# ShenhanQian/GaussianAvatars

Hardware: NVIDIA H100
Metric: rasterizer fwd+bwd frames/sec @100k splats 1080p (higher is better)
Workload: dtype f32

## Files before the change

gaussianavatars_b200/csrc/blend.cu:

```cuda
#include <type_traits>

#include "common.cuh"
#include "kernels.cuh"

namespace gab {

#define LOG2E 1.4426950408889634f
#define ALPHA_MIN (1.0f / 255.0f)
#define FULLMASK 0xffffffffu
#define CONIC_UNSCALE_AC (-2.0f / LOG2E)
#define CONIC_UNSCALE_B (-1.0f / LOG2E)

__device__ __forceinline__ float ex2_approx(float x) {
  float y;
  asm("ex2.approx.ftz.f32 %0, %1;" : "=f"(y) : "f"(x));
  return y;
}
__device__ __forceinline__ float rcp_approx(float x) {
  float y;
  asm("rcp.approx.ftz.f32 %0, %1;" : "=f"(y) : "f"(x));
  return y;
}
__device__ __forceinline__ void cp_async16(void* smem_dst, const void* gmem_src) {
  const unsigned s = (unsigned)__cvta_generic_to_shared(smem_dst);
  asm volatile("cp.async.cg.shared.global [%0], [%1], 16;" ::"r"(s), "l"(gmem_src) : "memory");
}
__device__ __forceinline__ void cp_async_commit() { asm volatile("cp.async.commit_group;" ::: "memory"); }
template <int N>
__device__ __forceinline__ void cp_async_wait() {
  asm volatile("cp.async.wait_group %0;" ::"n"(N) : "memory");
}
__device__ __forceinline__ void gather_rec(SplatRec* dst, const SplatRec* src) {
  cp_async16(&dst->q0, &src->q0);
  cp_async16(&dst->q1, &src->q1);
  cp_async16(&dst->q2, &src->q2);
}

__device__ __forceinline__ uint32_t smem_u32(const void* p) { return (uint32_t)__cvta_generic_to_shared(p); }
__device__ __forceinline__ void mbar_init(uint64_t* bar, uint32_t count) {
  asm volatile("mbarrier.init.shared::cta.b64 [%0], %1;" ::"r"(smem_u32(bar)), "r"(count) : "memory");
}
__device__ __forceinline__ void mbar_fence_init() { asm volatile("fence.mbarrier_init.release.cluster;" ::: "memory"); }
__device__ __forceinline__ void mbar_arrive_expect_tx(uint64_t* bar, uint32_t bytes) {
  asm volatile("mbarrier.arrive.expect_tx.shared::cta.b64 _, [%0], %1;" ::"r"(smem_u32(bar)), "r"(bytes) : "memory");
}
__device__ __forceinline__ void bulk_copy_g2s(void* smem_dst, const void* gmem_src, uint32_t bytes, uint64_t* bar) {
  asm volatile("cp.async.bulk.shared::cluster.global.mbarrier::complete_tx::bytes [%0], [%1], %2, [%3];" ::"r"(
                   smem_u32(smem_dst)),
               "l"(gmem_src), "r"(bytes), "r"(smem_u32(bar))
               : "memory");
}
__device__ __forceinline__ void mbar_wait(uint64_t* bar, uint32_t parity) {
  asm volatile(
      "{\n\t.reg .pred p;\n\tMBAR_WAIT:\n\tmbarrier.try_wait.parity.shared::cta.b64 p, [%0], %1;\n\t@p bra MBAR_DONE;\n\t"
      "bra MBAR_WAIT;\n\tMBAR_DONE:\n\t}" ::"r"(smem_u32(bar)),
      "r"(parity)
      : "memory");
}
#define GAB_FWD_DEPTH_CTAS 2
#define GAB_BWD_DEPTH_CTAS 5
#define ID_RING 3

template <int NT>
struct GroupBarrier {
  int id;
  __device__ __forceinline__ void sync() const { asm volatile("bar.sync %0, %1;" ::"r"(id), "n"(NT) : "memory"); }
  __device__ __forceinline__ bool sync_and(bool pred) const {
    unsigned r;
    asm volatile(
        "{\n\t.reg .pred p, q;\n\tsetp.ne.u32 q, %1, 0;\n\tbar.red.and.pred p, %2, %3, q;\n\tselp.u32 %0, 1, 0, p;\n\t}"
        : "=r"(r)
        : "r"((unsigned)pred), "r"(id), "n"(NT)
        : "memory");
    return r != 0;
  }
};

template <int K>
struct BandGeom {
  int col, row0, half, band0;
  __device__ __forceinline__ explicit BandGeom(int tl) {
    const int w = tl >> 5, lane = tl & 31;
    half = w & 1;
    band0 = (w >> 1) * K;
    col = half * 8 + (lane & 7);
    row0 = band0 * 4 + (lane >> 3);
  }
  __device__ __forceinline__ int bit(int i) const { return 2 * (band0 + i) + half; }
};

#define BLEND_OUT_FLOAT 1
#define BLEND_OUT_U8 2
__device__ __forceinline__ uint32_t quantize_u8(float c) {
  return __float2uint_rz(fminf(fmaxf(__fadd_rn(__fmul_rn(c, 255.f), 0.5f), 0.f), 255.f));
}
__device__ __forceinline__ void store_display(uint8_t* __restrict__ out, int W, int H, int pixx, int y, int lane,
                                              float r, float g, float b) {
  const uint32_t px = quantize_u8(r) | (quantize_u8(g) << 8) | (quantize_u8(b) << 16);
  const int j = lane & 7, x0 = pixx - j;
  const int p0 = min((4 * j) / 3, 6);
  const uint32_t lo = __shfl_sync(FULLMASK, px, (lane & ~7) | p0);
  const uint32_t hi = __shfl_sync(FULLMASK, px, (lane & ~7) | (p0 + 1));
  const uint32_t word = (uint32_t)((((uint64_t)hi << 24) | lo) >> (8 * (4 * j - 3 * p0)));
  if (y >= H) return;
  const size_t row = (size_t)y * W;
  if ((W & 3) == 0 && x0 + 8 <= W && ((uintptr_t)out & 3u) == 0) {
    if (j < 6) reinterpret_cast<uint32_t*>(out)[(row + x0) / 4 * 3 + j] = word;
  } else if (pixx < W) {
    uint8_t* o = out + (row + pixx) * 3;
    o[0] = (uint8_t)px;
    o[1] = (uint8_t)(px >> 8);
    o[2] = (uint8_t)(px >> 16);
  }
}

template <int K, int OUT, bool DA = false>
__device__ __forceinline__ void forward_tile(int tile, int tl, GroupBarrier<256 / K> bar, SplatRec* buf0,
                                             SplatRec* buf1, uint32_t* smask, uint32_t* ids_ring, uint64_t* mbar,
                                             int W, int H, int gx,
                                             const uint2* __restrict__ ranges, const uint32_t* __restrict__ point_list,
                                             const SplatRec* __restrict__ rec, const float* __restrict__ bg,
                                             float* __restrict__ out_color, float* __restrict__ final_T,
                                             uint32_t* __restrict__ n_contrib, uint8_t* __restrict__ strip_mask,
                                             uint8_t* __restrict__ out_rgb8, float* __restrict__ out_alpha = nullptr,
                                             float* __restrict__ out_depth = nullptr) {
  constexpr int NT = 256 / K;
  const int tx = tile % gx, ty = tile / gx;
  const int lane = tl & 31;
  const BandGeom<K> geo(tl);
  const int pixx = tx * GAB_TILE + geo.col;
  const int pixy0 = ty * GAB_TILE + geo.row0;
  const float fx = (float)pixx;
  float fy[K];
#pragma unroll
  for (int i = 0; i < K; i++) fy[i] = (float)(pixy0 + 4 * i);
  const uint2 range = ranges[tile];
  const int n = (int)(range.y - range.x);
  const uint32_t* ids = point_list + range.x;
  const bool want_mask = strip_mask != nullptr;
  smask[tl] = 0;

  float T[K], Cr[K], Cg[K], Cb[K];
  float D[DA ? K : 1];
  uint32_t last[K];
  uint32_t done = 0;
  constexpr uint32_t ALL = (1u << K) - 1u;
#pragma unroll
  for (int i = 0; i < K; i++) {
    T[i] = 1.f; Cr[i] = Cg[i] = Cb[i] = 0.f; last[i] = 0;
    if (DA) D[i] = 0.f;
    if (pixx >= W || pixy0 + 4 * i >= H) done |= 1u << i;
  }

  const int nchunks = (n + NT - 1) / NT;
  constexpr int RING_STRIDE = NT + 4;
  constexpr uint32_t CHUNK_BYTES = RING_STRIDE * 4;
  const int mis = (int)(range.x & 3u);
  const uint32_t* ids_al = ids - mis;
  if (tl == 0) {
#pragma unroll
    for (int k = 0; k < ID_RING; k++) mbar_init(&mbar[k], 1);
    mbar_fence_init();
  }
  bar.sync();
  auto issue_ids = [&](int k) {
    uint64_t* b = &mbar[k % ID_RING];
    mbar_arrive_expect_tx(b, CHUNK_BYTES);
    bulk_copy_g2s(ids_ring + (k % ID_RING) * RING_STRIDE, ids_al + (size_t)k * NT, CHUNK_BYTES, b);
  };
  auto wait_ids = [&](int k) { mbar_wait(&mbar[k % ID_RING], (uint32_t)((k / ID_RING) & 1)); };
  if (tl == 0) {
    if (nchunks > 0) issue_ids(0);
    if (nchunks > 1) issue_ids(1);
  }
  if (nchunks > 0) {
    wait_ids(0);
    if (tl < n) gather_rec(&buf0[tl], rec + ids_ring[mis + tl]);
  }
  cp_async_commit();

  for (int c = 0; c < nchunks; c++) {
    SplatRec* nxt = ((c + 1) & 1) ? buf1 : buf0;
    if (c + 1 < nchunks) {
      wait_ids(c + 1);
      const int p = (c + 1) * NT + tl;
      if (p < n) gather_rec(&nxt[tl], rec + ids_ring[((c + 1) % ID_RING) * RING_STRIDE + mis + tl]);
    }
    cp_async_commit();
    if (tl == 0 && c + 2 < nchunks) issue_ids(c + 2);
    cp_async_wait<1>();
    if (bar.sync_and(done == ALL)) {
      if (c + 2 < nchunks) wait_ids(c + 2);
      break;
    }
    const SplatRec* cur = (c & 1) ? buf1 : buf0;
    const int cnt = min(NT, n - c * NT);
    const uint32_t pos0 = (uint32_t)(c * NT);
    uint32_t lb[K];
#pragma unroll
    for (int i = 0; i < K; i++) lb[i] = 0;
    for (int gbase = 0; gbase < cnt; gbase += 32) {
      const int gend = min(32, cnt - gbase);
#pragma unroll 4
      for (int jj = 0; jj < gend; jj++) {
        const SplatRec* r = cur + gbase + jj;
        const float4 q0 = r->q0;
        const float4 q1 = r->q1;
        const float dx = q0.x - fx;
        const float tA = q0.z * dx;
#pragma unroll
        for (int i = 0; i < K; i++) {
          const float dy = q0.y - fy[i];
          const float pw = fmaf(q1.x * dy, dy, fmaf(q0.w, dy, tA) * dx);
          const float alpha = fminf(0.99f, q1.y * ex2_approx(pw));
          if (pw <= 0.f && alpha >= ALPHA_MIN && !((done >> i) & 1u)) {
            const float test_T = T[i] * (1.f - alpha);
            if (test_T < 0.0001f) {
              done |= 1u << i;
            } else {
              const float w = alpha * T[i];
              Cr[i] = fmaf(q1.z, w, Cr[i]);
              Cg[i] = fmaf(q1.w, w, Cg[i]);
              Cb[i] = fmaf(r->q2.x, w, Cb[i]);
              if (DA) D[i] = fmaf(r->q2.w, w, D[i]);
              T[i] = test_T;
              last[i] = pos0 + (uint32_t)(gbase + jj) + 1u;
              lb[i] |= 1u << jj;
            }
          }
        }
      }
      if (want_mask) {
        uint32_t wh = 0;
#pragma unroll
        for (int i = 0; i < K; i++) {
          const uint32_t rr = __reduce_or_sync(FULLMASK, lb[i]);
          wh |= ((rr >> lane) & 1u) << geo.bit(i);
          lb[i] = 0;
        }
        if (wh) atomicOr(&smask[gbase + lane], wh);
      }
      if (__all_sync(FULLMASK, done == ALL)) break;
    }
    bar.sync();
    if (want_mask && tl < cnt) {
      strip_mask[range.x + (uint32_t)(c * NT + tl)] = (uint8_t)smask[tl];
      smask[tl] = 0;
    }
  }
  cp_async_wait<0>();

  const float bg0 = bg[0], bg1 = bg[1], bg2 = bg[2];
  const size_t HW = (size_t)H * W;
#pragma unroll
  for (int i = 0; i < K; i++) {
    const int y = pixy0 + 4 * i;
    if (pixx < W && y < H) {
      const size_t pix = (size_t)y * W + pixx;
      if (OUT & BLEND_OUT_FLOAT) {
        out_color[pix] = fmaf(T[i], bg0, Cr[i]);
        out_color[HW + pix] = fmaf(T[i], bg1, Cg[i]);
        out_color[2 * HW + pix] = fmaf(T[i], bg2, Cb[i]);
      }
      if (final_T != nullptr) {
        final_T[pix] = T[i];
        n_contrib[pix] = last[i];
      }
      if (DA) {
        if (out_alpha != nullptr) out_alpha[pix] = 1.0f - T[i];
        if (out_depth != nullptr) out_depth[pix] = D[i];
      }
    }
  }
  if (OUT & BLEND_OUT_U8) {
#pragma unroll
    for (int i = 0; i < K; i++)
      store_display(out_rgb8, W, H, pixx, pixy0 + 4 * i, lane, fmaf(T[i], bg0, Cr[i]), fmaf(T[i], bg1, Cg[i]),
                    fmaf(T[i], bg2, Cb[i]));
  }
}

template <int KH, int OUT>
__global__ void __launch_bounds__(256) blend_forward_kernel(int W, int H, int gx, int tiles,
                                                            const uint2* __restrict__ ranges,
                                                            const uint32_t* __restrict__ order,
                                                            const uint32_t* __restrict__ order_info,
                                                            const uint32_t* __restrict__ point_list,
                                                            const SplatRec* __restrict__ rec,
                                                            const float* __restrict__ bg, float* __restrict__ out_color,
                                                            float* __restrict__ final_T,
                                                            uint32_t* __restrict__ n_contrib,
                                                            uint8_t* __restrict__ strip_mask,
                                                            uint8_t* __restrict__ out_rgb8) {
  __shared__ SplatRec buf[2][256];
  __shared__ uint32_t smask[256];
  __shared__ __align__(16) uint32_t ids_ring[4][ID_RING * (64 + 4)];
  __shared__ __align__(8) uint64_t mbar[4][ID_RING];
  constexpr int GH = KH;
  constexpr int NTH = 256 / KH;
  const int nh = (int)order_info[0];
  const int heavy_ctas = (nh + GH - 1) / GH;
  const int b = blockIdx.x, t = threadIdx.x;
  if (b < heavy_ctas) {
    const int g = t / NTH, slot = b * GH + g;
    if (slot >= nh) return;
    forward_tile<KH, OUT>((int)order[slot], t - g * NTH, GroupBarrier<NTH>{GH == 1 ? 0 : 1 + g}, buf[0] + g * NTH,
                          buf[1] + g * NTH, smask + g * NTH, &ids_ring[0][0] + g * (ID_RING * (NTH + 4)), mbar[g], W,
                          H, gx, ranges, point_list, rec, bg, out_color, final_T, n_contrib, strip_mask, out_rgb8);
  } else {
    const int g = t >> 6, slot = nh + 4 * (b - heavy_ctas) + g;
    if (slot >= tiles) return;
    forward_tile<4, OUT>((int)order[slot], t & 63, GroupBarrier<64>{1 + g}, buf[0] + g * 64, buf[1] + g * 64,
                         smask + g * 64, ids_ring[g], mbar[g], W, H, gx, ranges, point_list, rec, bg, out_color,
                         final_T, n_contrib, strip_mask, out_rgb8);
  }
}

void launch_blend_forward(int W, int H, const uint2* ranges, const uint32_t* order, const uint32_t* order_info,
                          const uint32_t* point_list, const SplatRec* rec, const float* bg, float* out_color,
                          float* final_T, uint32_t* n_contrib, uint8_t* strip_mask, uint8_t* out_rgb8,
                          cudaStream_t stream) {
  const int gx = (W + GAB_TILE - 1) / GAB_TILE, gy = (H + GAB_TILE - 1) / GAB_TILE;
  const int tiles = gx * gy;
  if (tiles == 0) return;
  const int grid = tiles;
  auto kernel = out_rgb8 == nullptr ? blend_forward_kernel<1, BLEND_OUT_FLOAT>
                : out_color == nullptr ? blend_forward_kernel<1, BLEND_OUT_U8>
                                       : blend_forward_kernel<1, BLEND_OUT_FLOAT | BLEND_OUT_U8>;
  kernel<<<grid, 256, 0, stream>>>(W, H, gx, tiles, ranges, order, order_info, point_list, rec, bg, out_color, final_T,
                                   n_contrib, strip_mask, out_rgb8);
  count_launch();
}

template <int OUT>
__global__ void __launch_bounds__(256, GAB_FWD_DEPTH_CTAS) blend_forward_depth_kernel(int W, int H, int gx, int tiles,
                                                                  const uint2* __restrict__ ranges,
                                                                  const uint32_t* __restrict__ order,
                                                                  const uint32_t* __restrict__ order_info,
                                                                  const uint32_t* __restrict__ point_list,
                                                                  const SplatRec* __restrict__ rec,
                                                                  const float* __restrict__ bg,
                                                                  float* __restrict__ out_color,
                                                                  float* __restrict__ final_T,
                                                                  uint32_t* __restrict__ n_contrib,
                                                                  uint8_t* __restrict__ strip_mask,
                                                                  uint8_t* __restrict__ out_rgb8,
                                                                  float* __restrict__ out_alpha,
                                                                  float* __restrict__ out_depth) {
  __shared__ SplatRec buf[2][256];
  __shared__ uint32_t smask[256];
  __shared__ __align__(16) uint32_t ids_ring[4][ID_RING * (64 + 4)];
  __shared__ __align__(8) uint64_t mbar[4][ID_RING];
  const int nh = (int)order_info[0];
  const int b = blockIdx.x, t = threadIdx.x;
  if (b < nh) {
    forward_tile<1, OUT, true>((int)order[b], t, GroupBarrier<256>{0}, buf[0], buf[1], smask, &ids_ring[0][0], mbar[0],
                               W, H, gx, ranges, point_list, rec, bg, out_color, final_T, n_contrib, strip_mask,
                               out_rgb8, out_alpha, out_depth);
  } else {
    const int g = t >> 6, slot = nh + 4 * (b - nh) + g;
    if (slot >= tiles) return;
    forward_tile<4, OUT, true>((int)order[slot], t & 63, GroupBarrier<64>{1 + g}, buf[0] + g * 64, buf[1] + g * 64,
                               smask + g * 64, ids_ring[g], mbar[g], W, H, gx, ranges, point_list, rec, bg, out_color,
                               final_T, n_contrib, strip_mask, out_rgb8, out_alpha, out_depth);
  }
}

void launch_blend_forward_depth(int W, int H, const uint2* ranges, const uint32_t* order, const uint32_t* order_info,
                                const uint32_t* point_list, const SplatRec* rec, const float* bg, float* out_color,
                                float* final_T, uint32_t* n_contrib, uint8_t* strip_mask, uint8_t* out_rgb8,
                                float* out_alpha, float* out_depth, cudaStream_t stream) {
  const int gx = (W + GAB_TILE - 1) / GAB_TILE, gy = (H + GAB_TILE - 1) / GAB_TILE;
  const int tiles = gx * gy;
  if (tiles == 0) return;
  auto kernel = out_rgb8 == nullptr ? blend_forward_depth_kernel<BLEND_OUT_FLOAT>
                : out_color == nullptr ? blend_forward_depth_kernel<BLEND_OUT_U8>
                                       : blend_forward_depth_kernel<BLEND_OUT_FLOAT | BLEND_OUT_U8>;
  kernel<<<tiles, 256, 0, stream>>>(W, H, gx, tiles, ranges, order, order_info, point_list, rec, bg, out_color, final_T,
                                    n_contrib, strip_mask, out_rgb8, out_alpha, out_depth);
  count_launch();
}

template <int OUT>
__global__ void __launch_bounds__(256) blend_forward_views_kernel(int W, int H, int gx, int tiles, int view_tiles,
                                                                  const uint2* __restrict__ ranges,
                                                                  const uint32_t* __restrict__ order,
                                                                  const uint32_t* __restrict__ order_info,
                                                                  const uint32_t* __restrict__ point_list,
                                                                  const SplatRec* __restrict__ rec,
                                                                  const float* __restrict__ bg,
                                                                  float* __restrict__ out_color,
                                                                  uint8_t* __restrict__ out_rgb8) {
  __shared__ SplatRec buf[2][256];
  __shared__ uint32_t smask[256];
  __shared__ __align__(16) uint32_t ids_ring[4][ID_RING * (64 + 4)];
  __shared__ __align__(8) uint64_t mbar[4][ID_RING];
  const int nh = (int)order_info[0];
  const int b = blockIdx.x, t = threadIdx.x;
  const bool heavy = b < nh;
  const int g = heavy ? 0 : t >> 6;
  const int slot = heavy ? b : nh + 4 * (b - nh) + g;
  if (slot >= (heavy ? nh : tiles)) return;
  const int tile = (int)order[slot];
  const int view = tile / view_tiles, local = tile - view * view_tiles;
  const size_t HW = (size_t)H * W;
  float* color = (OUT & BLEND_OUT_FLOAT) ? out_color + (size_t)view * 3 * HW : nullptr;
  uint8_t* rgb8 = (OUT & BLEND_OUT_U8) ? out_rgb8 + (size_t)view * 3 * HW : nullptr;
  const uint2* view_ranges = ranges + (size_t)view * view_tiles;
  if (heavy)
    forward_tile<1, OUT>(local, t, GroupBarrier<256>{0}, buf[0], buf[1], smask, &ids_ring[0][0], mbar[0], W, H, gx,
                         view_ranges, point_list, rec, bg, color, nullptr, nullptr, nullptr, rgb8);
  else
    forward_tile<4, OUT>(local, t & 63, GroupBarrier<64>{1 + g}, buf[0] + g * 64, buf[1] + g * 64, smask + g * 64,
                         ids_ring[g], mbar[g], W, H, gx, view_ranges, point_list, rec, bg, color, nullptr, nullptr,
                         nullptr, rgb8);
}

void launch_blend_forward_views(int views, int W, int H, const uint2* ranges, const uint32_t* order,
                                const uint32_t* order_info, const uint32_t* point_list, const SplatRec* rec,
                                const float* bg, float* out_color, uint8_t* out_rgb8, cudaStream_t stream) {
  const int gx = (W + GAB_TILE - 1) / GAB_TILE, gy = (H + GAB_TILE - 1) / GAB_TILE;
  const int view_tiles = gx * gy, tiles = views * view_tiles;
  if (tiles == 0) return;
  auto kernel = out_rgb8 == nullptr ? blend_forward_views_kernel<BLEND_OUT_FLOAT>
                : out_color == nullptr ? blend_forward_views_kernel<BLEND_OUT_U8>
                                       : blend_forward_views_kernel<BLEND_OUT_FLOAT | BLEND_OUT_U8>;
  kernel<<<tiles, 256, 0, stream>>>(W, H, gx, tiles, view_tiles, ranges, order, order_info, point_list, rec, bg,
                                    out_color, out_rgb8);
  count_launch();
}

__global__ void __launch_bounds__(256) blend_forward_views_train_kernel(int W, int H, int gx, int tiles, int view_tiles,
                                                                        const uint2* __restrict__ ranges,
                                                                        const uint32_t* __restrict__ order,
                                                                        const uint32_t* __restrict__ order_info,
                                                                        const uint32_t* __restrict__ point_list,
                                                                        const SplatRec* __restrict__ rec,
                                                                        const float* __restrict__ bg,
                                                                        float* __restrict__ out_color,
                                                                        float* __restrict__ final_T,
                                                                        uint32_t* __restrict__ n_contrib,
                                                                        uint8_t* __restrict__ strip_mask) {
  __shared__ SplatRec buf[2][256];
  __shared__ uint32_t smask[256];
  __shared__ __align__(16) uint32_t ids_ring[4][ID_RING * (64 + 4)];
  __shared__ __align__(8) uint64_t mbar[4][ID_RING];
  const int nh = (int)order_info[0];
  const int b = blockIdx.x, t = threadIdx.x;
  const bool heavy = b < nh;
  const int g = heavy ? 0 : t >> 6;
  const int slot = heavy ? b : nh + 4 * (b - nh) + g;
  if (slot >= (heavy ? nh : tiles)) return;
  const int tile = (int)order[slot];
  const int view = tile / view_tiles, local = tile - view * view_tiles;
  const size_t HW = (size_t)H * W;
  float* color = out_color + (size_t)view * 3 * HW;
  float* vT = final_T + (size_t)view * HW;
  uint32_t* vn = n_contrib + (size_t)view * HW;
  const uint2* view_ranges = ranges + (size_t)view * view_tiles;
  if (heavy)
    forward_tile<1, BLEND_OUT_FLOAT>(local, t, GroupBarrier<256>{0}, buf[0], buf[1], smask, &ids_ring[0][0], mbar[0], W,
                                     H, gx, view_ranges, point_list, rec, bg, color, vT, vn, strip_mask, nullptr);
  else
    forward_tile<4, BLEND_OUT_FLOAT>(local, t & 63, GroupBarrier<64>{1 + g}, buf[0] + g * 64, buf[1] + g * 64,
                                     smask + g * 64, ids_ring[g], mbar[g], W, H, gx, view_ranges, point_list, rec, bg,
                                     color, vT, vn, strip_mask, nullptr);
}

void launch_blend_forward_views_train(int views, int W, int H, const uint2* ranges, const uint32_t* order,
                                      const uint32_t* order_info, const uint32_t* point_list, const SplatRec* rec,
                                      const float* bg, float* out_color, float* final_T, uint32_t* n_contrib,
                                      uint8_t* strip_mask, cudaStream_t stream) {
  const int gx = (W + GAB_TILE - 1) / GAB_TILE, gy = (H + GAB_TILE - 1) / GAB_TILE;
  const int view_tiles = gx * gy, tiles = views * view_tiles;
  if (tiles == 0) return;
  blend_forward_views_train_kernel<<<tiles, 256, 0, stream>>>(W, H, gx, tiles, view_tiles, ranges, order, order_info,
                                                              point_list, rec, bg, out_color, final_T, n_contrib,
                                                              strip_mask);
  count_launch();
}

template <int OUT>
__global__ void __launch_bounds__(256, GAB_FWD_DEPTH_CTAS) blend_forward_views_depth_kernel(
    int W, int H, int gx, int tiles, int view_tiles, const uint2* __restrict__ ranges, const uint32_t* __restrict__ order,
    const uint32_t* __restrict__ order_info, const uint32_t* __restrict__ point_list, const SplatRec* __restrict__ rec,
    const float* __restrict__ bg, float* __restrict__ out_color, float* __restrict__ final_T,
    uint32_t* __restrict__ n_contrib, uint8_t* __restrict__ strip_mask, uint8_t* __restrict__ out_rgb8,
    float* __restrict__ out_alpha, float* __restrict__ out_depth) {
  __shared__ SplatRec buf[2][256];
  __shared__ uint32_t smask[256];
  __shared__ __align__(16) uint32_t ids_ring[4][ID_RING * (64 + 4)];
  __shared__ __align__(8) uint64_t mbar[4][ID_RING];
  const int nh = (int)order_info[0];
  const int b = blockIdx.x, t = threadIdx.x;
  const bool heavy = b < nh;
  const int g = heavy ? 0 : t >> 6;
  const int slot = heavy ? b : nh + 4 * (b - nh) + g;
  if (slot >= (heavy ? nh : tiles)) return;
  const int tile = (int)order[slot];
  const int view = tile / view_tiles, local = tile - view * view_tiles;
  const size_t HW = (size_t)H * W, off = (size_t)view * HW;
  float* color = (OUT & BLEND_OUT_FLOAT) ? out_color + 3 * off : nullptr;
  uint8_t* rgb8 = (OUT & BLEND_OUT_U8) ? out_rgb8 + 3 * off : nullptr;
  float* vT = final_T != nullptr ? final_T + off : nullptr;
  uint32_t* vn = final_T != nullptr ? n_contrib + off : nullptr;
  float* va = out_alpha != nullptr ? out_alpha + off : nullptr;
  float* vd = out_depth != nullptr ? out_depth + off : nullptr;
  const uint2* view_ranges = ranges + (size_t)view * view_tiles;
  if (heavy)
    forward_tile<1, OUT, true>(local, t, GroupBarrier<256>{0}, buf[0], buf[1], smask, &ids_ring[0][0], mbar[0], W, H,
                               gx, view_ranges, point_list, rec, bg, color, vT, vn, strip_mask, rgb8, va, vd);
  else
    forward_tile<4, OUT, true>(local, t & 63, GroupBarrier<64>{1 + g}, buf[0] + g * 64, buf[1] + g * 64,
                               smask + g * 64, ids_ring[g], mbar[g], W, H, gx, view_ranges, point_list, rec, bg, color,
                               vT, vn, strip_mask, rgb8, va, vd);
}

void launch_blend_forward_views_depth(int views, int W, int H, const uint2* ranges, const uint32_t* order,
                                      const uint32_t* order_info, const uint32_t* point_list, const SplatRec* rec,
                                      const float* bg, float* out_color, float* final_T, uint32_t* n_contrib,
                                      uint8_t* strip_mask, uint8_t* out_rgb8, float* out_alpha, float* out_depth,
                                      cudaStream_t stream) {
  const int gx = (W + GAB_TILE - 1) / GAB_TILE, gy = (H + GAB_TILE - 1) / GAB_TILE;
  const int view_tiles = gx * gy, tiles = views * view_tiles;
  if (tiles == 0) return;
  auto kernel = out_rgb8 == nullptr ? blend_forward_views_depth_kernel<BLEND_OUT_FLOAT>
                : out_color == nullptr ? blend_forward_views_depth_kernel<BLEND_OUT_U8>
                                       : blend_forward_views_depth_kernel<BLEND_OUT_FLOAT | BLEND_OUT_U8>;
  kernel<<<tiles, 256, 0, stream>>>(W, H, gx, tiles, view_tiles, ranges, order, order_info, point_list, rec, bg,
                                    out_color, final_T, n_contrib, strip_mask, out_rgb8, out_alpha, out_depth);
  count_launch();
}

template <int K>
struct PixState {
  float fy[K];
  float T[K];
  float ar[K], ag[K], ab[K];
  float dr[K], dg[K], db[K];
  float bgT[K];
  int nc[K];
};
struct SplatSums {
  float S0, S1, S2, go, gr, gg, gb;
};
template <int K>
struct PixStateDA : PixState<K> {
  float az[K];
  float dD[K];
};
struct SplatSumsDA : SplatSums {
  float gz;
};
template <int K, bool DA>
using PixStateT = std::conditional_t<DA, PixStateDA<K>, PixState<K>>;
template <bool DA>
using SplatSumsT = std::conditional_t<DA, SplatSumsDA, SplatSums>;

template <int K, int M, bool DA = false>
__device__ __forceinline__ void visit_bands(PixStateT<K, DA>& p, int pos, float py, float tA, float dx, float Bp,
                                            float Cp, float op, float cr, float cg, float cb, SplatSumsT<DA>& s,
                                            float cz = 0.f) {
#pragma unroll
  for (int i = 0; i < K; i++) {
    if (!((M >> i) & 1)) continue;
    const float dy = py - p.fy[i];
    const float pw = fmaf(Cp * dy, dy, fmaf(Bp, dy, tA) * dx);
    const float G = ex2_approx(pw);
    const float alpha = fminf(0.99f, op * G);
    const bool valid = pos < p.nc[i] && pw <= 0.f && alpha >= ALPHA_MIN;
    const float al = valid ? alpha : 0.f;
    const float Gv = valid ? G : 0.f;
    const float ra = valid ? rcp_approx(1.f - alpha) : 1.f;
    const float Tn = p.T[i] * ra;
    p.T[i] = Tn;
    const float w = al * Tn;
    s.gr = fmaf(w, p.dr[i], s.gr);
    s.gg = fmaf(w, p.dg[i], s.gg);
    s.gb = fmaf(w, p.db[i], s.gb);
    const float er = cr - p.ar[i], eg = cg - p.ag[i], eb = cb - p.ab[i];
    float dLda = er * p.dr[i];
    dLda = fmaf(eg, p.dg[i], dLda);
    dLda = fmaf(eb, p.db[i], dLda);
    float ez = 0.f;
    if constexpr (DA) {
      ez = cz - p.az[i];
      dLda = fmaf(ez, p.dD[i], dLda);
      s.gz = fmaf(w, p.dD[i], s.gz);
    }
    dLda = fmaf(dLda, Tn, -p.bgT[i] * ra);
    p.ar[i] = fmaf(al, er, p.ar[i]);
    p.ag[i] = fmaf(al, eg, p.ag[i]);
    p.ab[i] = fmaf(al, eb, p.ab[i]);
    if constexpr (DA) p.az[i] = fmaf(al, ez, p.az[i]);
    const float t = Gv * dLda;
    s.go += t;
    const float s_ = op * t;
    const float sd = s_ * dy;
    s.S0 += s_;
    s.S1 += sd;
    s.S2 = fmaf(sd, dy, s.S2);
  }
}

template <int K, int I, bool DA = false>
struct BandLoop {
  static __device__ __forceinline__ void run(uint32_t m, PixStateT<K, DA>& p, int pos, float py, float tA, float dx,
                                             float Bp, float Cp, float op, float cr, float cg, float cb,
                                             SplatSumsT<DA>& s, float cz = 0.f) {
    if (m & (1u << I)) visit_bands<K, (1 << I), DA>(p, pos, py, tA, dx, Bp, Cp, op, cr, cg, cb, s, cz);
    BandLoop<K, I + 1, DA>::run(m, p, pos, py, tA, dx, Bp, Cp, op, cr, cg, cb, s, cz);
  }
};
template <int K, bool DA>
struct BandLoop<K, K, DA> {
  static __device__ __forceinline__ void run(uint32_t, PixStateT<K, DA>&, int, float, float, float, float, float, float,
                                             float, float, float, SplatSumsT<DA>&, float = 0.f) {}
};

#define ROWS_STRIDE 36
template <int NR>
struct __align__(16) WarpSmemT {
  SplatRec rec[2][32];
  float rows[2][NR * ROWS_STRIDE];
  float part[2][32];
  uint32_t ids[ID_RING][32 + 4];
  uint8_t masks[ID_RING][32 + 16];
  uint64_t mbar[ID_RING];
};
using WarpSmem = WarpSmemT<9>;

template <int K, bool DA = false>
__device__ __forceinline__ void backward_task(int tile, int tl, WarpSmemT<DA ? 10 : 9>& sm, int W, int H, int gx,
                                              const uint2* __restrict__ ranges,
                                              const uint32_t* __restrict__ point_list,
                                              const SplatRec* __restrict__ rec, const float* __restrict__ bg,
                                              const float* __restrict__ final_T,
                                              const uint32_t* __restrict__ n_contrib,
                                              const float* __restrict__ dL_dpix,
                                              const uint8_t* __restrict__ strip_mask, float* __restrict__ g2d,
                                              const float* __restrict__ dL_dalpha = nullptr,
                                              const float* __restrict__ dL_ddepth = nullptr) {
  constexpr int NR = DA ? 10 : 9;
  const int tx = tile % gx, ty = tile / gx;
  const int lane = tl & 31;
  const BandGeom<K> geo(tl);
  const int pixx = tx * GAB_TILE + geo.col;
  const int pixy0 = ty * GAB_TILE + geo.row0;
  const float fx = (float)pixx;
  const uint2 range = ranges[tile];
  const size_t HW = (size_t)H * W;
  const float bg0 = bg[0], bg1 = bg[1], bg2 = bg[2];

  PixStateT<K, DA> p;
  int n = 0;
#pragma unroll
  for (int i = 0; i < K; i++) {
    const int y = pixy0 + 4 * i;
    p.fy[i] = (float)y;
    p.ar[i] = p.ag[i] = p.ab[i] = 0.f;
    float T0 = 0.f, dr = 0.f, dg = 0.f, db = 0.f, dA = 0.f, dZ = 0.f;
    p.nc[i] = 0;
    if (pixx < W && y < H) {
      const size_t pix = (size_t)y * W + pixx;
      T0 = final_T[pix];
      p.nc[i] = (int)n_contrib[pix];
      dr = dL_dpix[pix];
      dg = dL_dpix[HW + pix];
      db = dL_dpix[2 * HW + pix];
      if constexpr (DA) {
        if (dL_dalpha != nullptr) dA = dL_dalpha[pix];
        if (dL_ddepth != nullptr) dZ = dL_ddepth[pix];
      }
    }
    p.T[i] = T0;
    p.dr[i] = dr;
    p.dg[i] = dg;
    p.db[i] = db;
    if constexpr (DA) {
      p.bgT[i] = T0 * ((bg0 * dr + bg1 * dg + bg2 * db) - dA);
      p.az[i] = 0.f;
      p.dD[i] = dZ;
// ... 280 lines not shown
```

Baseline: 1723.

## Restructure forward blend into per-warp tasks with warp-local staging

Replaces CTA/group-level tile processing (named barriers, 256-thread blocks, shared smask staging) with per-warp tasks: each warp owns its own id ring, mbarriers and 32-splat double buffer, synchronising only with __syncwarp. Blocks shrink to 128 threads with higher occupancy bounds, heavy tiles are split across warp pairs with K=2, and strip_mask bits are combined via shuffles and written with global atomicOr. This is meant to remove block-wide barrier stalls and let warps retire early independently. The cost is more global atomics, smaller per-fetch chunks, and more frequent id-ring/mbarrier traffic per warp.

```diff
diff --git a/gaussianavatars_b200/csrc/blend.cu b/gaussianavatars_b200/csrc/blend.cu
--- a/gaussianavatars_b200/csrc/blend.cu
+++ b/gaussianavatars_b200/csrc/blend.cu
@@ -57,24 +57,10 @@
       "r"(parity)
       : "memory");
 }
-#define GAB_FWD_DEPTH_CTAS 2
+#define GAB_FWD_CTAS 6
+#define GAB_FWD_DEPTH_CTAS 5
 #define GAB_BWD_DEPTH_CTAS 5
 #define ID_RING 3
-
-template <int NT>
-struct GroupBarrier {
-  int id;
-  __device__ __forceinline__ void sync() const { asm volatile("bar.sync %0, %1;" ::"r"(id), "n"(NT) : "memory"); }
-  __device__ __forceinline__ bool sync_and(bool pred) const {
-    unsigned r;
-    asm volatile(
-        "{\n\t.reg .pred p, q;\n\tsetp.ne.u32 q, %1, 0;\n\tbar.red.and.pred p, %2, %3, q;\n\tselp.u32 %0, 1, 0, p;\n\t}"
-        : "=r"(r)
-        : "r"((unsigned)pred), "r"(id), "n"(NT)
-        : "memory");
-    return r != 0;
-  }
-};
 
 template <int K>
 struct BandGeom {
@@ -114,17 +100,20 @@
   }
 }
 
+struct __align__(16) FwdWarpSmem {
+  SplatRec rec[2][32];
+  uint32_t ids[ID_RING][32];
+  uint64_t mbar[ID_RING];
+};
+
 template <int K, int OUT, bool DA = false>
-__device__ __forceinline__ void forward_tile(int tile, int tl, GroupBarrier<256 / K> bar, SplatRec* buf0,
-                                             SplatRec* buf1, uint32_t* smask, uint32_t* ids_ring, uint64_t* mbar,
-                                             int W, int H, int gx,
+__device__ __forceinline__ void forward_task(int tile, int tl, FwdWarpSmem& sm, int W, int H, int gx,
                                              const uint2* __restrict__ ranges, const uint32_t* __restrict__ point_list,
                                              const SplatRec* __restrict__ rec, const float* __restrict__ bg,
                                              float* __restrict__ out_color, float* __restrict__ final_T,
                                              uint32_t* __restrict__ n_contrib, uint8_t* __restrict__ strip_mask,
                                              uint8_t* __restrict__ out_rgb8, float* __restrict__ out_alpha = nullptr,
                                              float* __restrict__ out_depth = nullptr) {
-  constexpr int NT = 256 / K;
   const int tx = tile % gx, ty = tile / gx;
   const int lane = tl & 31;
   const BandGeom<K> geo(tl);
@@ -136,9 +125,8 @@
   for (int i = 0; i < K; i++) fy[i] = (float)(pixy0 + 4 * i);
   const uint2 range = ranges[tile];
   const int n = (int)(range.y - range.x);
-  const uint32_t* ids = point_list + range.x;
-  const bool want_mask = strip_mask != nullptr;
-  smask[tl] = 0;
+  const uint32_t start = range.x & ~3u;
+  const int mis = (int)(range.x - start);
 
   float T[K], Cr[K], Cg[K], Cb[K];
   float D[DA ? K : 1];
@@ -151,101 +139,93 @@
     if (DA) D[i] = 0.f;
     if (pixx >= W || pixy0 + 4 * i >= H) done |= 1u << i;
   }
-
-  const int nchunks = (n + NT - 1) / NT;
-  constexpr int RING_STRIDE = NT + 4;
-  constexpr uint32_t CHUNK_BYTES = RING_STRIDE * 4;
-  const int mis = (int)(range.x & 3u);
-  const uint32_t* ids_al = ids - mis;
-  if (tl == 0) {
-#pragma unroll
-    for (int k = 0; k < ID_RING; k++) mbar_init(&mbar[k], 1);
+  const bool idle = __all_sync(FULLMASK, done == ALL);
+  const int nchunks = (n == 0 || idle) ? 0 : (n + mis + 31) >> 5;
+
+  constexpr uint32_t CHUNK_BYTES = 32 * 4;
+  if (lane == 0) {
+#pragma unroll
+    for (int k = 0; k < ID_RING; k++) mbar_init(&sm.mbar[k], 1);
     mbar_fence_init();
   }
-  bar.sync();
+  __syncwarp();
   auto issue_ids = [&](int k) {
-    uint64_t* b = &mbar[k % ID_RING];
+    uint64_t* b = &sm.mbar[k % ID_RING];
     mbar_arrive_expect_tx(b, CHUNK_BYTES);
-    bulk_copy_g2s(ids_ring + (k % ID_RING) * RING_STRIDE, ids_al + (size_t)k * NT, CHUNK_BYTES, b);
+    bulk_copy_g2s(sm.ids[k % ID_RING], point_list + start + (uint32_t)k * 32u, CHUNK_BYTES, b);
   };
-  auto wait_ids = [&](int k) { mbar_wait(&mbar[k % ID_RING], (uint32_t)((k / ID_RING) & 1)); };
-  if (tl == 0) {
+  auto wait_ids = [&](int k) { mbar_wait(&sm.mbar[k % ID_RING], (uint32_t)((k / ID_RING) & 1)); };
+  auto gather_chunk = [&](int k) {
+    wait_ids(k);
+    const int j = k * 32 + lane - mis;
+    if (j >= 0 && j < n) gather_rec(&sm.rec[k & 1][lane], rec + sm.ids[k % ID_RING][lane]);
+    cp_async_commit();
+  };
+  if (lane == 0) {
     if (nchunks > 0) issue_ids(0);
     if (nchunks > 1) issue_ids(1);
   }
-  if (nchunks > 0) {
-    wait_ids(0);
-    if (tl < n) gather_rec(&buf0[tl], rec + ids_ring[mis + tl]);
-  }
-  cp_async_commit();
-
+  if (nchunks > 0) gather_chunk(0);
+
+  const bool want_mask = strip_mask != nullptr;
   for (int c = 0; c < nchunks; c++) {
-    SplatRec* nxt = ((c + 1) & 1) ? buf1 : buf0;
-    if (c + 1 < nchunks) {
-      wait_ids(c + 1);
-      const int p = (c + 1) * NT + tl;
-      if (p < n) gather_rec(&nxt[tl], rec + ids_ring[((c + 1) % ID_RING) * RING_STRIDE + mis + tl]);
-    }
-    cp_async_commit();
-    if (tl == 0 && c + 2 < nchunks) issue_ids(c + 2);
+    __syncwarp();
+    if (c + 1 < nchunks) gather_chunk(c + 1);
+    else cp_async_commit();
+    if (lane == 0 && c + 2 < nchunks) issue_ids(c + 2);
     cp_async_wait<1>();
-    if (bar.sync_and(done == ALL)) {
-      if (c + 2 < nchunks) wait_ids(c + 2);
-      break;
-    }
-    const SplatRec* cur = (c & 1) ? buf1 : buf0;
-    const int cnt = min(NT, n - c * NT);
-    const uint32_t pos0 = (uint32_t)(c * NT);
+    __syncwarp();
+    const SplatRec* cur = sm.rec[c & 1];
+    const int base = c * 32 - mis;
+    const int j0 = max(0, -base), j1 = min(32, n - base);
     uint32_t lb[K];
 #pragma unroll
     for (int i = 0; i < K; i++) lb[i] = 0;
-    for (int gbase = 0; gbase < cnt; gbase += 32) {
-      const int gend = min(32, cnt - gbase);
 #pragma unroll 4
-      for (int jj = 0; jj < gend; jj++) {
-        const SplatRec* r = cur + gbase + jj;
-        const float4 q0 = r->q0;
-        const float4 q1 = r->q1;
-        const float dx = q0.x - fx;
-        const float tA = q0.z * dx;
-#pragma unroll
-        for (int i = 0; i < K; i++) {
-          const float dy = q0.y - fy[i];
-          const float pw = fmaf(q1.x * dy, dy, fmaf(q0.w, dy, tA) * dx);
-          const float alpha = fminf(0.99f, q1.y * ex2_approx(pw));
-          if (pw <= 0.f && alpha >= ALPHA_MIN && !((done >> i) & 1u)) {
-            const float test_T = T[i] * (1.f - alpha);
-            if (test_T < 0.0001f) {
-              done |= 1u << i;
-            } else {
-              const float w = alpha * T[i];
-              Cr[i] = fmaf(q1.z, w, Cr[i]);
-              Cg[i] = fmaf(q1.w, w, Cg[i]);
-              Cb[i] = fmaf(r->q2.x, w, Cb[i]);
-              if (DA) D[i] = fmaf(r->q2.w, w, D[i]);
-              T[i] = test_T;
-              last[i] = pos0 + (uint32_t)(gbase + jj) + 1u;
-              lb[i] |= 1u << jj;
-            }
+    for (int jj = j0; jj < j1; jj++) {
+      const SplatRec* r = cur + jj;
+      const float4 q0 = r->q0;
+      const float4 q1 = r->q1;
+      const float dx = q0.x - fx;
+      const float tA = q0.z * dx;
+#pragma unroll
+      for (int i = 0; i < K; i++) {
+        const float dy = q0.y - fy[i];
+        const float pw = fmaf(q1.x * dy, dy, fmaf(q0.w, dy, tA) * dx);
+        const float alpha = fminf(0.99f, q1.y * ex2_approx(pw));
+        if (pw <= 0.f && alpha >= ALPHA_MIN && !((done >> i) & 1u)) {
+          const float test_T = T[i] * (1.f - alpha);
+          if (test_T < 0.0001f) {
+            done |= 1u << i;
+          } else {
+            const float w = alpha * T[i];
+            Cr[i] = fmaf(q1.z, w, Cr[i]);
+            Cg[i] = fmaf(q1.w, w, Cg[i]);
+            Cb[i] = fmaf(r->q2.x, w, Cb[i]);
+            if (DA) D[i] = fmaf(r->q2.w, w, D[i]);
+            T[i] = test_T;
+            last[i] = (uint32_t)(base + jj) + 1u;
+            lb[i] |= 1u << jj;
           }
         }
       }
-      if (want_mask) {
-        uint32_t wh = 0;
-#pragma unroll
-        for (int i = 0; i < K; i++) {
-          const uint32_t rr = __reduce_or_sync(FULLMASK, lb[i]);
-          wh |= ((rr >> lane) & 1u) << geo.bit(i);
-          lb[i] = 0;
-        }
-        if (wh) atomicOr(&smask[gbase + lane], wh);
+    }
+    if (want_mask) {
+      uint32_t wh = 0;
+#pragma unroll
+      for (int i = 0; i < K; i++) {
+        const uint32_t rr = __reduce_or_sync(FULLMASK, lb[i]);
+        wh |= ((rr >> lane) & 1u) << geo.bit(i);
       }
-      if (__all_sync(FULLMASK, done == ALL)) break;
+      uint32_t word = wh << (8 * (lane & 3));
+      word |= __shfl_xor_sync(FULLMASK, word, 1);
+      word |= __shfl_xor_sync(FULLMASK, word, 2);
+      uint32_t* words = reinterpret_cast<uint32_t*>(strip_mask + start);
+      if ((lane & 3) == 0 && word != 0u) atomicOr(&words[c * 8 + (lane >> 2)], word);
     }
-    bar.sync();
-    if (want_mask && tl < cnt) {
-      strip_mask[range.x + (uint32_t)(c * NT + tl)] = (uint8_t)smask[tl];
-      smask[tl] = 0;
+    if (__all_sync(FULLMASK, done == ALL)) {
+      if (c + 2 < nchunks) wait_ids(c + 2);
+      break;
     }
   }
   cp_async_wait<0>();
@@ -280,40 +260,36 @@
   }
 }
 
-template <int KH, int OUT>
-__global__ void __launch_bounds__(256) blend_forward_kernel(int W, int H, int gx, int tiles,
-                                                            const uint2* __restrict__ ranges,
-                                                            const uint32_t* __restrict__ order,
-                                                            const uint32_t* __restrict__ order_info,
-                                                            const uint32_t* __restrict__ point_list,
-                                                            const SplatRec* __restrict__ rec,
-                                                            const float* __restrict__ bg, float* __restrict__ out_color,
-                                                            float* __restrict__ final_T,
-                                                            uint32_t* __restrict__ n_contrib,
-                                                            uint8_t* __restrict__ strip_mask,
-                                                            uint8_t* __restrict__ out_rgb8) {
-  __shared__ SplatRec buf[2][256];
-  __shared__ uint32_t smask[256];
-  __shared__ __align__(16) uint32_t ids_ring[4][ID_RING * (64 + 4)];
-  __shared__ __align__(8) uint64_t mbar[4][ID_RING];
-  constexpr int GH = KH;
-  constexpr int NTH = 256 / KH;
-  const int nh = (int)order_info[0];
-  const int heavy_ctas = (nh + GH - 1) / GH;
-  const int b = blockIdx.x, t = threadIdx.x;
-  if (b < heavy_ctas) {
-    const int g = t / NTH, slot = b * GH + g;
-    if (slot >= nh) return;
-    forward_tile<KH, OUT>((int)order[slot], t - g * NTH, GroupBarrier<NTH>{GH == 1 ? 0 : 1 + g}, buf[0] + g * NTH,
-                          buf[1] + g * NTH, smask + g * NTH, &ids_ring[0][0] + g * (ID_RING * (NTH + 4)), mbar[g], W,
-                          H, gx, ranges, point_list, rec, bg, out_color, final_T, n_contrib, strip_mask, out_rgb8);
-  } else {
-    const int g = t >> 6, slot = nh + 4 * (b - heavy_ctas) + g;
-    if (slot >= tiles) return;
-    forward_tile<4, OUT>((int)order[slot], t & 63, GroupBarrier<64>{1 + g}, buf[0] + g * 64, buf[1] + g * 64,
-                         smask + g * 64, ids_ring[g], mbar[g], W, H, gx, ranges, point_list, rec, bg, out_color,
-                         final_T, n_contrib, strip_mask, out_rgb8);
-  }
+struct FwdSlot {
+  int slot;
+  bool heavy;
+  __device__ __forceinline__ FwdSlot(int nh, int b, int w) : slot(b < nh ? b : nh + 2 * (b - nh) + (w >> 1)),
+                                                             heavy(b < nh) {}
+};
+
+template <int OUT>
+__global__ void __launch_bounds__(128, GAB_FWD_CTAS) blend_forward_kernel(int W, int H, int gx, int tiles,
+                                                                          const uint2* __restrict__ ranges,
+                                                                          const uint32_t* __restrict__ order,
+                                                                          const uint32_t* __restrict__ order_info,
+                                                                          const uint32_t* __restrict__ point_list,
+                                                                          const SplatRec* __restrict__ rec,
+                                                                          const float* __restrict__ bg,
+                                                                          float* __restrict__ out_color,
+                                                                          float* __restrict__ final_T,
+                                                                          uint32_t* __restrict__ n_contrib,
+                                                                          uint8_t* __restrict__ strip_mask,
+                                                                          uint8_t* __restrict__ out_rgb8) {
+  __shared__ FwdWarpSmem sm[4];
+  const int t = threadIdx.x, w = t >> 5;
+  const FwdSlot s((int)order_info[0], blockIdx.x, w);
+  if (s.slot >= tiles) return;
+  if (s.heavy)
+    forward_task<2, OUT>((int)order[s.slot], t, sm[w], W, H, gx, ranges, point_list, rec, bg, out_color, final_T,
+                         n_contrib, strip_mask, out_rgb8);
+  else
+    forward_task<4, OUT>((int)order[s.slot], t & 63, sm[w], W, H, gx, ranges, point_list, rec, bg, out_color, final_T,
+                         n_contrib, strip_mask, out_rgb8);
 }
 
 void launch_blend_forward(int W, int H, const uint2* ranges, const uint32_t* order, const uint32_t* order_info,
@@ -323,17 +299,16 @@
   const int gx = (W + GAB_TILE - 1) / GAB_TILE, gy = (H + GAB_TILE - 1) / GAB_TILE;
   const int tiles = gx * gy;
   if (tiles == 0) return;
-  const int grid = tiles;
-  auto kernel = out_rgb8 == nullptr ? blend_forward_kernel<1, BLEND_OUT_FLOAT>
-                : out_color == nullptr ? blend_forward_kernel<1, BLEND_OUT_U8>
-                                       : blend_forward_kernel<1, BLEND_OUT_FLOAT | BLEND_OUT_U8>;
-  kernel<<<grid, 256, 0, stream>>>(W, H, gx, tiles, ranges, order, order_info, point_list, rec, bg, out_color, final_T,
-                                   n_contrib, strip_mask, out_rgb8);
+  auto kernel = out_rgb8 == nullptr ? blend_forward_kernel<BLEND_OUT_FLOAT>
+                : out_color == nullptr ? blend_forward_kernel<BLEND_OUT_U8>
+                                       : blend_forward_kernel<BLEND_OUT_FLOAT | BLEND_OUT_U8>;
+  kernel<<<tiles, 128, 0, stream>>>(W, H, gx, tiles, ranges, order, order_info, point_list, rec, bg, out_color, final_T,
+                                    n_contrib, strip_mask, out_rgb8);
   count_launch();
 }
 
 template <int OUT>
-__global__ void __launch_bounds__(256, GAB_FWD_DEPTH_CTAS) blend_forward_depth_kernel(int W, int H, int gx, int tiles,
+__global__ void __launch_bounds__(128, GAB_FWD_DEPTH_CTAS) blend_forward_depth_kernel(int W, int H, int gx, int tiles,
                                                                   const uint2* __restrict__ ranges,
                                                                   const uint32_t* __restrict__ order,
                                                                   const uint32_t* __restrict__ order_info,
@@ -347,23 +322,16 @@
                                                                   uint8_t* __restrict__ out_rgb8,
                                                                   float* __restrict__ out_alpha,
                                                                   float* __restrict__ out_depth) {
-  __shared__ SplatRec buf[2][256];
-  __shared__ uint32_t smask[256];
-  __shared__ __align__(16) uint32_t ids_ring[4][ID_RING * (64 + 4)];
-  __shared__ __align__(8) uint64_t mbar[4][ID_RING];
-  const int nh = (int)order_info[0];
-  const int b = blockIdx.x, t = threadIdx.x;
-  if (b < nh) {
-    forward_tile<1, OUT, true>((int)order[b], t, GroupBarrier<256>{0}, buf[0], buf[1], smask, &ids_ring[0][0], mbar[0],
-                               W, H, gx, ranges, point_list, rec, bg, out_color, final_T, n_contrib, strip_mask,
-                               out_rgb8, out_alpha, out_depth);
-  } else {
-    const int g = t >> 6, slot = nh + 4 * (b - nh) + g;
-    if (slot >= tiles) return;
-    forward_tile<4, OUT, true>((int)order[slot], t & 63, GroupBarrier<64>{1 + g}, buf[0] + g * 64, buf[1] + g * 64,
-                               smask + g * 64, ids_ring[g], mbar[g], W, H, gx, ranges, point_list, rec, bg, out_color,
+  __shared__ FwdWarpSmem sm[4];
+  const int t = threadIdx.x, w = t >> 5;
+  const FwdSlot s((int)order_info[0], blockIdx.x, w);
+  if (s.slot >= tiles) return;
+  if (s.heavy)
+    forward_task<2, OUT, true>((int)order[s.slot], t, sm[w], W, H, gx, ranges, point_list, rec, bg, out_color, final_T,
+                               n_contrib, strip_mask, out_rgb8, out_alpha, out_depth);
+  else
+    forward_task<4, OUT, true>((int)order[s.slot], t & 63, sm[w], W, H, gx, ranges, point_list, rec, bg, out_color,
                                final_T, n_contrib, strip_mask, out_rgb8, out_alpha, out_depth);
-  }
 }
 
 void launch_blend_forward_depth(int W, int H, const uint2* ranges, const uint32_t* order, const uint32_t* order_info,
@@ -376,43 +344,37 @@
   auto kernel = out_rgb8 == nullptr ? blend_forward_depth_kernel<BLEND_OUT_FLOAT>
                 : out_color == nullptr ? blend_forward_depth_kernel<BLEND_OUT_U8>
                                        : blend_forward_depth_kernel<BLEND_OUT_FLOAT | BLEND_OUT_U8>;
-  kernel<<<tiles, 256, 0, stream>>>(W, H, gx, tiles, ranges, order, order_info, point_list, rec, bg, out_color, final_T,
+  kernel<<<tiles, 128, 0, stream>>>(W, H, gx, tiles, ranges, order, order_info, point_list, rec, bg, out_color, final_T,
                                     n_contrib, strip_mask, out_rgb8, out_alpha, out_depth);
   count_launch();
 }
 
 template <int OUT>
-__global__ void __launch_bounds__(256) blend_forward_views_kernel(int W, int H, int gx, int tiles, int view_tiles,
-                                                                  const uint2* __restrict__ ranges,
-                                                                  const uint32_t* __restrict__ order,
-                                                                  const uint32_t* __restrict__ order_info,
-                                                                  const uint32_t* __restrict__ point_list,
-                                                                  const SplatRec* __restrict__ rec,
-                                                                  const float* __restrict__ bg,
-                                                                  float* __restrict__ out_color,
-                                                                  uint8_t* __restrict__ out_rgb8) {
-  __shared__ SplatRec buf[2][256];
-  __shared__ uint32_t smask[256];
-  __shared__ __align__(16) uint32_t ids_ring[4][ID_RING * (64 + 4)];
-  __shared__ __align__(8) uint64_t mbar[4][ID_RING];
-  const int nh = (int)order_info[0];
-  const int b = blockIdx.x, t = threadIdx.x;
-  const bool heavy = b < nh;
-  const int g = heavy ? 0 : t >> 6;
-  const int slot = heavy ? b : nh + 4 * (b - nh) + g;
-  if (slot >= (heavy ? nh : tiles)) return;
-  const int tile = (int)order[slot];
+__global__ void __launch_bounds__(128, GAB_FWD_CTAS) blend_forward_views_kernel(int W, int H, int gx, int tiles,
+                                                                                int view_tiles,
+                                                                                const uint2* __restrict__ ranges,
+                                                                                const uint32_t* __restrict__ order,
+                                                                                const uint32_t* __restrict__ order_info,
+                                                                                const uint32_t* __restrict__ point_list,
+                                                                                const SplatRec* __restrict__ rec,
+                                                                                const float* __restrict__ bg,
+                                                                                float* __restrict__ out_color,
+                                                                                uint8_t* __restrict__ out_rgb8) {
+  __shared__ FwdWarpSmem sm[4];
+  const int t = threadIdx.x, w = t >> 5;
+  const FwdSlot s((int)order_info[0], blockIdx.x, w);
+  if (s.slot >= tiles) return;
+  const int tile = (int)order[s.slot];
   const int view = tile / view_tiles, local = tile - view * view_tiles;
   const size_t HW = (size_t)H * W;
   float* color = (OUT & BLEND_OUT_FLOAT) ? out_color + (size_t)view * 3 * HW : nullptr;
   uint8_t* rgb8 = (OUT & BLEND_OUT_U8) ? out_rgb8 + (size_t)view * 3 * HW : nullptr;
   const uint2* view_ranges = ranges + (size_t)view * view_tiles;
-  if (heavy)
-    forward_tile<1, OUT>(local, t, GroupBarrier<256>{0}, buf[0], buf[1], smask, &ids_ring[0][0], mbar[0], W, H, gx,
-                         view_ranges, point_list, rec, bg, color, nullptr, nullptr, nullptr, rgb8);
+  if (s.heavy)
+    forward_task<2, OUT>(local, t, sm[w], W, H, gx, view_ranges, point_list, rec, bg, color, nullptr, nullptr, nullptr,
+                         rgb8);
   else
-    forward_tile<4, OUT>(local, t & 63, GroupBarrier<64>{1 + g}, buf[0] + g * 64, buf[1] + g * 64, smask + g * 64,
-                         ids_ring[g], mbar[g], W, H, gx, view_ranges, point_list, rec, bg, color, nullptr, nullptr,
+    forward_task<4, OUT>(local, t & 63, sm[w], W, H, gx, view_ranges, point_list, rec, bg, color, nullptr, nullptr,
                          nullptr, rgb8);
 }
 
@@ -425,46 +387,33 @@
   auto kernel = out_rgb8 == nullptr ? blend_forward_views_kernel<BLEND_OUT_FLOAT>
                 : out_color == nullptr ? blend_forward_views_kernel<BLEND_OUT_U8>
                                        : blend_forward_views_kernel<BLEND_OUT_FLOAT | BLEND_OUT_U8>;
-  kernel<<<tiles, 256, 0, stream>>>(W, H, gx, tiles, view_tiles, ranges, order, order_info, point_list, rec, bg,
+  kernel<<<tiles, 128, 0, stream>>>(W, H, gx, tiles, view_tiles, ranges, order, order_info, point_list, rec, bg,
                                     out_color, out_rgb8);
   count_launch();
 }
 
-__global__ void __launch_bounds__(256) blend_forward_views_train_kernel(int W, int H, int gx, int tiles, int view_tiles,
-                                                                        const uint2* __restrict__ ranges,
-                                                                        const uint32_t* __restrict__ order,
-                                                                        const uint32_t* __restrict__ order_info,
-                                                                        const uint32_t* __restrict__ point_list,
-                                                                        const SplatRec* __restrict__ rec,
-                                                                        const float* __restrict__ bg,
-                                                                        float* __restrict__ out_color,
-                                                                        float* __restrict__ final_T,
-                                                                        uint32_t* __restrict__ n_contrib,
-                                                                        uint8_t* __restrict__ strip_mask) {
-  __shared__ SplatRec buf[2][256];
-  __shared__ uint32_t smask[256];
-  __shared__ __align__(16) uint32_t ids_ring[4][ID_RING * (64 + 4)];
-  __shared__ __align__(8) uint64_t mbar[4][ID_RING];
-  const int nh = (int)order_info[0];
-  const int b = blockIdx.x, t = threadIdx.x;
-  const bool heavy = b < nh;
-  const int g = heavy ? 0 : t >> 6;
-  const int slot = heavy ? b : nh + 4 * (b - nh) + g;
-  if (slot >= (heavy ? nh : tiles)) return;
-  const int tile = (int)order[slot];
+__global__ void __launch_bounds__(128, GAB_FWD_CTAS) blend_forward_views_train_kernel(
+    int W, int H, int gx, int tiles, int view_tiles, const uint2* __restrict__ ranges, const uint32_t* __restrict__ order,
+    const uint32_t* __restrict__ order_info, const uint32_t* __restrict__ point_list, const SplatRec* __restrict__ rec,
+    const float* __restrict__ bg, float* __restrict__ out_color, float* __restrict__ final_T,
+    uint32_t* __restrict__ n_contrib, uint8_t* __restrict__ strip_mask) {
+  __shared__ FwdWarpSmem sm[4];
+  const int t = threadIdx.x, w = t >> 5;
+  const FwdSlot s((int)order_info[0], blockIdx.x, w);
+  if (s.slot >= tiles) return;
+  const int tile = (int)order[s.slot];
   const int view = tile / view_tiles, local = tile - view * view_tiles;
   const size_t HW = (size_t)H * W;
   float* color = out_color + (size_t)view * 3 * HW;
   float* vT = final_T + (size_t)view * HW;
   uint32_t* vn = n_contrib + (size_t)view * HW;
   const uint2* view_ranges = ranges + (size_t)view * view_tiles;
-  if (heavy)
-    forward_tile<1, BLEND_OUT_FLOAT>(local, t, GroupBarrier<256>{0}, buf[0], buf[1], smask, &ids_ring[0][0], mbar[0], W,
-                                     H, gx, view_ranges, point_list, rec, bg, color, vT, vn, strip_mask, nullptr);
+  if (s.heavy)
+    forward_task<2, BLEND_OUT_FLOAT>(local, t, sm[w], W, H, gx, view_ranges, point_list, rec, bg, color, vT, vn,
+                                     strip_mask, nullptr);
   else
-    forward_tile<4, BLEND_OUT_FLOAT>(local, t & 63, GroupBarrier<64>{1 + g}, buf[0] + g * 64, buf[1] + g * 64,
-                                     smask + g * 64, ids_ring[g], mbar[g], W, H, gx, view_ranges, point_list, rec, bg,
-                                     color, vT, vn, strip_mask, nullptr);
+    forward_task<4, BLEND_OUT_FLOAT>(local, t & 63, sm[w], W, H, gx, view_ranges, point_list, rec, bg, color, vT, vn,
+                                     strip_mask, nullptr);
 }
 
 void launch_blend_forward_views_train(int views, int W, int H, const uint2* ranges, const uint32_t* order,
@@ -474,30 +423,24 @@
   const int gx = (W + GAB_TILE - 1) / GAB_TILE, gy = (H + GAB_TILE - 1) / GAB_TILE;
   const int view_tiles = gx * gy, tiles = views * view_tiles;
   if (tiles == 0) return;
-  blend_forward_views_train_kernel<<<tiles, 256, 0, stream>>>(W, H, gx, tiles, view_tiles, ranges, order, order_info,
+  blend_forward_views_train_kernel<<<tiles, 128, 0, stream>>>(W, H, gx, tiles, view_tiles, ranges, order, order_info,
                                                               point_list, rec, bg, out_color, final_T, n_contrib,
                                                               strip_mask);
   count_launch();
 }
 
 template <int OUT>
-__global__ void __launch_bounds__(256, GAB_FWD_DEPTH_CTAS) blend_forward_views_depth_kernel(
+__global__ void __launch_bounds__(128, GAB_FWD_DEPTH_CTAS) blend_forward_views_depth_kernel(
     int W, int H, int gx, int tiles, int view_tiles, const uint2* __restrict__ ranges, const uint32_t* __restrict__ order,
     const uint32_t* __restrict__ order_info, const uint32_t* __restrict__ point_list, const SplatRec* __restrict__ rec,
     const float* __restrict__ bg, float* __restrict__ out_color, float* __restrict__ final_T,
     uint32_t* __restrict__ n_contrib, uint8_t* __restrict__ strip_mask, uint8_t* __restrict__ out_rgb8,
     float* __restrict__ out_alpha, float* __restrict__ out_depth) {
-  __shared__ SplatRec buf[2][256];
-  __shared__ uint32_t smask[256];
-  __shared__ __align__(16) uint32_t ids_ring[4][ID_RING * (64 + 4)];
-  __shared__ __align__(8) uint64_t mbar[4][ID_RING];
-  const int nh = (int)order_info[0];
-  const int b = blockIdx.x, t = threadIdx.x;
-  const bool heavy = b < nh;
-  const int g = heavy ? 0 : t >> 6;
-  const int slot = heavy ? b : nh + 4 * (b - nh) + g;
-  if (slot >= (heavy ? nh : tiles)) return;
-  const int tile = (int)order[slot];
+  __shared__ FwdWarpSmem sm[4];
+  const int t = threadIdx.x, w = t >> 5;
+  const FwdSlot s((int)order_info[0], blockIdx.x, w);
+  if (s.slot >= tiles) return;
+  const int tile = (int)order[s.slot];
   const int view = tile / view_tiles, local = tile - view * view_tiles;
   const size_t HW = (size_t)H * W, off = (size_t)view * HW;
   float* color = (OUT & BLEND_OUT_FLOAT) ? out_color + 3 * off : nullptr;
@@ -507,13 +450,12 @@
   float* va = out_alpha != nullptr ? out_alpha + off : nullptr;
   float* vd = out_depth != nullptr ? out_depth + off : nullptr;
   const uint2* view_ranges = ranges + (size_t)view * view_tiles;
-  if (heavy)
-    forward_tile<1, OUT, true>(local, t, GroupBarrier<256>{0}, buf[0], buf[1], smask, &ids_ring[0][0], mbar[0], W, H,
-                               gx, view_ranges, point_list, rec, bg, color, vT, vn, strip_mask, rgb8, va, vd);
+  if (s.heavy)
+    forward_task<2, OUT, true>(local, t, sm[w], W, H, gx, view_ranges, point_list, rec, bg, color, vT, vn, strip_mask,
+                               rgb8, va, vd);
   else
-    forward_tile<4, OUT, true>(local, t & 63, GroupBarrier<64>{1 + g}, buf[0] + g * 64, buf[1] + g * 64,
-                               smask + g * 64, ids_ring[g], mbar[g], W, H, gx, view_ranges, point_list, rec, bg, color,
-                               vT, vn, strip_mask, rgb8, va, vd);
+    forward_task<4, OUT, true>(local, t & 63, sm[w], W, H, gx, view_ranges, point_list, rec, bg, color, vT, vn,
+                               strip_mask, rgb8, va, vd);
 }
 
 void launch_blend_forward_views_depth(int views, int W, int H, const uint2* ranges, const uint32_t* order,
@@ -527,7 +469,7 @@
   auto kernel = out_rgb8 == nullptr ? blend_forward_views_depth_kernel<BLEND_OUT_FLOAT>
                 : out_color == nullptr ? blend_forward_views_depth_kernel<BLEND_OUT_U8>
                                        : blend_forward_views_depth_kernel<BLEND_OUT_FLOAT | BLEND_OUT_U8>;
-  kernel<<<tiles, 256, 0, stream>>>(W, H, gx, tiles, view_tiles, ranges, order, order_info, point_list, rec, bg,
+  kernel<<<tiles, 128, 0, stream>>>(W, H, gx, tiles, view_tiles, ranges, order, order_info, point_list, rec, bg,
                                     out_color, final_T, n_contrib, strip_mask, out_rgb8, out_alpha, out_depth);
   count_launch();
 }
```

Result: faster. 1800, median of 6 (+4.4%).
